# faverogian/diffusion-classifier

Measured on AMD Instinct MI355X. Metric: images classified/sec (node), CIFAR-10 10-class x 50-step ELBO scoring, higher is better.
Workload: dtype bf16; 1 GPU; cifar10-unet-10x50; classes=10, trials=50, forwards_per_image=500, input=uniform [-1,1], parallelism=single

## Files before the change

diffusion-classifier_amd/csrc/conv3_halo.hip:

```cpp
#include <stdlib.h>
#include "common.h"
#ifdef DC_STAMPS
static __device__ unsigned long long* g_stamps;
extern "C" void dc_debug_set_stamps(unsigned long long* p) { (void)hipMemcpyToSymbol(HIP_SYMBOL(g_stamps), &p, sizeof(p)); }
#define DC_STAMP(k) do { if (threadIdx.x == 0 && g_stamps) g_stamps[blockIdx.x * 8 + (k)] = __builtin_amdgcn_s_memtime(); } while (0)
static __device__ int g_halo_abl;
extern "C" void dc_debug_set_halo_abl(int v) { (void)hipMemcpyToSymbol(HIP_SYMBOL(g_halo_abl), &v, sizeof(v)); }
#define DC_HALO_ABL() __builtin_amdgcn_readfirstlane(g_halo_abl)
#else
#define DC_STAMP(k) do {} while (0)
#define DC_HALO_ABL() 0
#endif
#include "igemm_epilogue.h"
#include "epi_pn.h"

static __device__ unsigned g_pn_timeouts;
static __device__ chunk16 g_zero_page[16];
#include "conv3_halo_plan.h"
DC_CLOCK_DECL(conv3_halo)

template <typename T, int NW, int NTAP = 9, int MODE = 0, bool STG = false, bool PN = false, typename... TL>
__global__ __launch_bounds__(NW * 64, 2) void conv3_halo_kernel(const IgemmArgs a, const HaloGeom g, const TL... tl) {
  constexpr bool TAIL = sizeof...(TL) == 1;
  static_assert(sizeof...(TL) <= 1 && (!TAIL || (PN && NW == 4 && NTAP == 9 && MODE == 1 && sizeof(T) == 2)), "tail fold: the 16-bit 4-wave exchange form");
  static_assert(!PN || (MODE == 1 && NW == 4 && !STG) || ((MODE == 0 || MODE == 2) && NW == 8 && STG && NTAP == 9), "producer-side GroupNorm: one-image-per-patch forms, or 8x8 / 4x4 images");
  constexpr bool PNX = PN && NW == 4, PNL = PN && NW == 8;
  static_assert(!STG || NW == 8, "staggered loop: the 8-wave kernel");
  constexpr bool XB = MODE == 1, MOS = MODE == 2;
  using Cfg = HaloCfg<NW>;
  constexpr int EPC = Elem<T>::EPC;
  constexpr int BKE = 4 * EPC;
  constexpr int TM = 8, TN = 4;
  constexpr int NT = Cfg::NT, WLD = Cfg::WLD, WR = Cfg::WR, PD = Cfg::WR - 1;
  extern __shared__ __attribute__((aligned(16))) char smem[];
  char* const Wring = smem + 2 * Cfg::XBUF;

  DC_STAMP(0);
  const int t = threadIdx.x;
  const int lane = t & 63;
  const int wave = __builtin_amdgcn_readfirstlane(t >> 6);
  const int wm = wave >> 1, wn = wave & 1;
  const int lr = lane & 15, lq = lane >> 4;
  int tile_m, tile_n;
  if constexpr (PNX) {
    constexpr int LPH = NTAP == 4 ? 2 : 0;
    const int tnr = a.tiles_n >> LPH;
    const int kq = blockIdx.x >> 3;
    const int grp = ((kq >> (g.lpt + LPH)) << 3) + (blockIdx.x & 7);
    if (grp >= g.n_img * tnr) return;
    const int smp = grp / tnr;
    const int within = kq & ((1 << (g.lpt + LPH)) - 1);
    tile_n = __builtin_amdgcn_readfirstlane((within >> g.lpt) * tnr + grp - smp * tnr);
    tile_m = __builtin_amdgcn_readfirstlane((smp << g.lpt) + (within & ((1 << g.lpt) - 1)));
    asm volatile("" : "+s"(tile_m), "+s"(tile_n));
  } else if constexpr (XB) tile_of_block_scalar(a, tile_m, tile_n);
  else tile_of_block(a, tile_m, tile_n);
  constexpr bool UP4 = NTAP == 4;
  int phase = 0;
  if (UP4) { const int tn = a.tiles_n >> 2; phase = tile_n / tn; tile_n -= phase * tn; }
  const int pa = phase >> 1, pb = phase & 1;
  int tx = tile_m % g.tiles_x;
  int ty = (tile_m / g.tiles_x) % g.tiles_y;
  int ng = tile_m / (g.tiles_x * g.tiles_y);
  const int tw = 1 << g.ltw, th = 1 << g.lth;
  const int HW = g.H * g.W;
  const int HWs = a.upsample ? (g.H >> 1) * (g.W >> 1) : HW;
  const int Ctot = a.C0 + a.C1;
  const int c0chunks = a.C0 / BKE, nchunks = Ctot / BKE;

  constexpr int NXL = Cfg::NXL;
  int pp[NXL];
  const int xlx = t & 3;
  int* const tbl = reinterpret_cast<int*>(smem + Cfg::TBLOFF);
  if (t < (1 << g.lni)) {
    const int n = (ng << g.lni) + t;
    const bool vn = n < g.n_img;
    tbl[4 * t] = vn ? (a.map0 ? a.map0[n] : n) * HWs : -1;
    tbl[4 * t + 1] = (vn && a.src1) ? (a.map1 ? a.map1[n] : n) * HWs : -1;
    tbl[4 * t + 2] = (vn && a.src2) ? (a.map2 ? a.map2[n] : n) * HWs : -1;
  }
  auto piece_code = [&](int i, int* col = nullptr) -> int {
    const int hr = (i * NT + t) >> 2;
    int code = -1;
    if (col) *col = 0;
    if (i < g.nxl && hr < g.HR) {
      if constexpr (MOS) {
        const int hy = (int)(((float)hr + 0.5f) * g.inv_hw), hx = hr - hy * g.hw;
        const int cy = (int)(((float)hy + 0.5f) * g.inv_ch), ry = hy - cy * (th + 1);
        const int cx = (int)(((float)hx + 0.5f) * g.inv_cw), rx = hx - cx * (tw + 1);
        if (col) *col = hx;
        if (ry > 0 && rx > 0) code = (((cy << g.lmc) + cx) << 20) | ((ry - 1) * g.W + rx - 1);
      } else {
        const int img = (int)(((float)hr + 0.5f) * g.inv_hp), r = hr - img * g.hp;
        const int hy = (int)(((float)r + 0.5f) * g.inv_hw), hx = r - hy * g.hw;
        const int iy = ty * th + hy - 1, ix = tx * tw + hx - 1;
        if (col) *col = hx;
        if ((unsigned)iy < (unsigned)g.H && (unsigned)ix < (unsigned)g.W)
          code = (img << 20) | (a.upsample ? (iy >> 1) * (g.W >> 1) + (ix >> 1) : iy * g.W + ix);
      }
    }
    return code;
  };
  constexpr bool SWP = !STG;
#pragma unroll
  for (int i = 0; i < NXL; ++i) {
    int col;
    pp[i] = piece_code(i, &col);
    if constexpr (SWP) { if (pp[i] >= 0) pp[i] |= ((col >> g.sws) & 1) << 30; }
  }
  auto sw_of = [&](int pk) -> int { if constexpr (SWP) return (pk >> 30) & 1; else return 0; };
  constexpr int PKMASK = SWP ? 0x3FFFFFFF : -1;
  float* const brv = reinterpret_cast<float*>(smem + Cfg::GNOFF);
  constexpr bool STAGE_BRV = XB;
  if (STAGE_BRV && t < 128) {
    const int c = tile_n * 128 + t;
    float v = 0.f;
    if (c < a.Cout) {
      if (a.bias) v = a.bias[c];
      if (a.rowvec) v += a.rowvec[(size_t)(a.rowvec_map ? a.rowvec_map[ng] : ng) * a.rowvec_ld + c];
    }
    brv[t] = v;
  }
  if constexpr (PNX) {
    if (t >= 128 && t < 256) {
      const int c = tile_n * 128 + t - 128;
      brv[t] = a.pn_gamma[c];
      brv[t + 128] = a.pn_beta[c];
    }
  }
  __syncthreads();
  const char* zero = reinterpret_cast<const char*>(g_zero_page);
  constexpr bool XROW = STG && !XB;
  auto retarget = [&](int which) {
#pragma unroll
    for (int i = 0; i < NXL; ++i) {
      const int code = piece_code(i);
      int row = -1;
      if (code >= 0) {
        const int b = tbl[4 * (code >> 20) + which];
        if (b >= 0) row = b + (code & 0xFFFFF);
      }
      pp[i] = row;
    }
  };
  if constexpr (XROW) retarget(0);

  const T* xb0 = nullptr; const T* xb1 = nullptr; const T* xb2 = nullptr;
  int wvoff = 0, ldb0 = 0, ldb1 = 0, ldb2 = 0;
  if (XB) {
    ldb0 = a.ld0 * (int)sizeof(T); ldb1 = a.ld1 * (int)sizeof(T); ldb2 = a.ld2 * (int)sizeof(T);
    asm volatile("" : "+s"(ldb0), "+s"(ldb1), "+s"(ldb2));
    const int n = ng;
    const int s0 = __builtin_amdgcn_readfirstlane(a.map0 ? a.map0[n] : n);
    xb0 = reinterpret_cast<const T*>(a.src0) + (size_t)s0 * HWs * a.ld0;
    if (a.src1) { const int s1 = __builtin_amdgcn_readfirstlane(a.map1 ? a.map1[n] : n); xb1 = reinterpret_cast<const T*>(a.src1) + (size_t)s1 * HWs * a.ld1; }
    if (a.src2) { const int s2 = __builtin_amdgcn_readfirstlane(a.map2 ? a.map2[n] : n); xb2 = reinterpret_cast<const T*>(a.src2) + (size_t)s2 * HWs * a.ld2; }
  }
  if (XB || STG) {
    const int wrow0 = t >> 2;
    wvoff = (epi_wrow(wrow0, false) * a.Ktot + ((t & 3) ^ swz64(wrow0)) * EPC) * (int)sizeof(T);
  }
  auto rsrc_of = [](const void* base) { return __builtin_amdgcn_make_buffer_rsrc(const_cast<void*>(base), 0, 0x7fffffff, 0x00020000); };

  auto issue_x = [&](int cc, int i0 = 0, int i1 = 64) {
    const int which = cc >= nchunks ? 2 : (cc >= c0chunks ? 1 : 0);
    if constexpr (XB) {
      int ldb = ldb0, cb = cc;
      const T* xb = xb0;
      if (cc >= nchunks) { ldb = ldb2; cb = cc - nchunks; xb = xb2; }
      else if (cc >= c0chunks) { ldb = ldb1; cb = cc - c0chunks; xb = xb1; }
      const int cofs = cb * 64 + xlx * 16;
      const __amdgpu_buffer_rsrc_t rs = rsrc_of(xb);
      char* xs = smem + (cc & 1) * Cfg::XBUF + wave * 1024;
#pragma unroll
      for (int i = 0; i < NXL; ++i) {
        if (i < i0 || i >= i1) continue;
        int pk = pp[i];
        asm volatile("" : "+v"(pk));
        const int voff = pk < 0 ? -1 : (pk & PKMASK) * ldb + (cofs ^ (sw_of(pk) << 5));
        __builtin_amdgcn_raw_ptr_buffer_load_lds(rs, (lptr_t)(xs + i * (NT * 16)), 16, voff, 0, 0, 0);
      }
      return;
    } else {
    const T* src = reinterpret_cast<const T*>(which == 2 ? a.src2 : (which == 1 ? a.src1 : a.src0));
    const int ld = which == 2 ? a.ld2 : (which == 1 ? a.ld1 : a.ld0);
    const int coff = (which == 2 ? cc - nchunks : (which == 1 ? cc - c0chunks : cc)) * BKE + xlx * EPC;
    char* xs = smem + (cc & 1) * Cfg::XBUF + wave * 1024;
#pragma unroll
    for (int i = 0; i < NXL; ++i) {
      if (i < i0 || i >= i1) continue;
      int pk = pp[i];
      asm volatile("" : "+v"(pk));
      int rowi;
      if constexpr (XROW) rowi = pk;
      else {
        const int base = pk < 0 ? -1 : tbl[4 * ((pk & PKMASK) >> 20) + which];
        rowi = base < 0 ? -1 : base + (pk & 0xFFFFF);
      }
      const size_t e = (size_t)(rowi < 0 ? 0 : rowi) * ld + (coff ^ (sw_of(pk) << 1) * EPC);
      const char* gp = rowi < 0 ? zero : reinterpret_cast<const char*>(src + e);
      __builtin_amdgcn_global_load_lds((gptr_t)gp, (lptr_t)(xs + i * (NT * 16)), 16, 0, 0);
    }
    }
  };
  const int wtile0 = ((UP4 ? phase * (a.tiles_n >> 2) : 0) + tile_n) * 128 * a.Ktot;
  auto issue_w = [&](int cc, int tap, int slot) {
    if constexpr (XB || STG) {
      const int so = (wtile0 + tap * Ctot + cc * BKE) * (int)sizeof(T);
      const __amdgpu_buffer_rsrc_t wrs = rsrc_of(a.W);
#pragma unroll
      for (int i = 0; i < WLD; ++i)
        __builtin_amdgcn_raw_ptr_buffer_load_lds(wrs, (lptr_t)(Wring + slot * HALO_WST + i * (NT * 16) + wave * 1024), 16, wvoff,
                                                 __builtin_amdgcn_readfirstlane(so + i * 64 * a.Ktot * (int)sizeof(T)), 0, 0);
    } else {
      const T* wb = reinterpret_cast<const T*>(a.W) + (size_t)wtile0 + (size_t)tap * Ctot + (size_t)cc * BKE;
      int tt = t;
      asm volatile("" : "+v"(tt));
#pragma unroll
      for (int i = 0; i < WLD; ++i) {
        const int row = (i * NT + tt) >> 2;
        const int wro = epi_wrow(row, false) * a.Ktot + ((tt & 3) ^ swz64(row)) * EPC;
        __builtin_amdgcn_global_load_lds((gptr_t) reinterpret_cast<const char*>(wb + wro),
                                         (lptr_t)(Wring + slot * HALO_WST + i * (NT * 16) + wave * 1024), 16, 0, 0);
      }
    }
  };

  auto issue_w2 = [&](int e, int slot) {
    int tt = t;
    asm volatile("" : "+v"(tt));
#pragma unroll
    for (int i = 0; i < WLD; ++i) {
      const int row = (i * NT + tt) >> 2;
      const T* wp = reinterpret_cast<const T*>(a.W2) + (size_t)(tile_n * 128 + epi_wrow(row, false)) * a.C2 + ((tt & 3) ^ swz64(row)) * EPC + e * BKE;
      __builtin_amdgcn_global_load_lds((gptr_t) reinterpret_cast<const char*>(wp),
                                       (lptr_t)(Wring + slot * HALO_WST + i * (NT * 16) + wave * 1024), 16, 0, 0);
    }
  };
  const int nx = a.src2 ? a.C2 / BKE : 0;

  constexpr int NV = 3;
  int xlv[NV];
  {
    const int xx = lr & ((tw < 16 ? tw : 16) - 1);
    const int rowpart = ((lr >> g.ltw) * g.hw + (lr & (tw - 1))) * 64;
#pragma unroll
    for (int k = 0; k < NV; ++k) xlv[k] = rowpart + ((lq ^ (SWP ? (((xx + k + (UP4 ? pb : 0)) >> g.sws) & 1) << 1 : 0)) << 4);
  }
  int joff[TM];
#pragma unroll
  for (int j = 0; j < TM; ++j) {
    const int p = wm * 128 + j * 16;
    const int img = p >> (g.ltw + g.lth), py = (p >> g.ltw) & (th - 1), px = p & (tw - 1);
    const int o = MOS ? ((img >> g.lmc) * (th + 1) + py) * g.hw + (img & ((1 << g.lmc) - 1)) * (tw + 1) + px : img * g.hp + py * g.hw + px;
    joff[j] = __builtin_amdgcn_readfirstlane(o * 64);
  }
  const int woff0 = lds64_off(wn * 64 + lr, lq);

  f32x4 acc[TN][TM];
#pragma unroll
  for (int i = 0; i < TN; ++i)
#pragma unroll
    for (int j = 0; j < TM; ++j) acc[i][j] = f32x4{0.f, 0.f, 0.f, 0.f};

  constexpr int XD = HALO_XDEPTH;
  static_assert(XD >= 2 && XD <= TM, "pixel-fragment ring: 2 ... TM quads");
  const uint32_t lds0 = lds_addr_of(smem);
  const uint32_t waddr = lds_addr_of(Wring) + (uint32_t)woff0;
  auto mma_tap = [&](uint32_t wso, uint32_t xbo, int tapoff, auto kxc) {
    constexpr int kx = decltype(kxc)::value;
    chunk16 wf[TN], xq[XD];
    const uint32_t xu = lds0 + xbo + (uint32_t)tapoff;
    auto xread = [&](int j) { return ds_read16_async(xu + (uint32_t)joff[j] + (uint32_t)xlv[MOS ? ((kx + j) & 1) : kx]); };
    __builtin_amdgcn_sched_barrier(0);
    const uint32_t wa = waddr + wso;
    wf[0] = ds_read16_async_off<0>(wa);
    wf[1] = ds_read16_async_off<1024>(wa);
    wf[2] = ds_read16_async_off<2048>(wa);
    wf[3] = ds_read16_async_off<3072>(wa);
#pragma unroll
    for (int j = 0; j < XD; ++j) xq[j] = xread(j);
    auto group = [&](auto jc) {
      constexpr int j = decltype(jc)::value, q = j % XD;
      constexpr int fly = (TM - 1 - j) < (XD - 1) ? (TM - 1 - j) : (XD - 1);
      if constexpr (j == 0) lgkm_wait<fly>(wf[0], wf[1], wf[2], wf[3], xq[0]);
      else lgkm_wait<fly>(xq[q]);
      __builtin_amdgcn_sched_barrier(0);
#pragma unroll
      for (int i = 0; i < TN; ++i) acc[i][j] = Mma<T>::run(wf[i], xq[q], acc[i][j]);
      __builtin_amdgcn_sched_barrier(0);
      if constexpr (j + XD < TM) xq[q] = xread(j + XD);
    };
    group(IC<0>{}); group(IC<1>{}); group(IC<2>{}); group(IC<3>{}); group(IC<4>{}); group(IC<5>{}); group(IC<6>{}); group(IC<7>{});
    __builtin_amdgcn_sched_barrier(0);
  };

  DC_STAMP(1);
  if constexpr (STG) {
    const bool grpB = wave >= 4;
    const int abl = DC_HALO_ABL();
    int cur_which = 0;
    issue_x(0);
#pragma unroll
    for (int i = 0; i < PD; ++i) issue_w(0, i, i);
    hwait_vmcnt<0>();
    __builtin_amdgcn_s_barrier();
    if (grpB) __builtin_amdgcn_s_barrier();
    DC_CLOCK(0);
    chunk16 wf[TN], xf[TM / 2];
    uint32_t xaddr[TM];
#pragma unroll
    for (int j = 0; j < TM; ++j) xaddr[j] = lds0 + (uint32_t)(joff[j] + xlv[0]);
    for (int cc = 0; cc < nchunks; ++cc) {
      const bool side_next = cc + 1 == nchunks && nx > 0;
      const bool has_next = cc + 1 < nchunks || side_next;
      const int s0 = cc * NTAP;
      const uint32_t xbo = (uint32_t)(cc & 1) * Cfg::XBUF;
      if constexpr (XROW) {
        const int wnext = cc + 1 >= nchunks ? 2 : (cc + 1 >= c0chunks ? 1 : 0);
        if (has_next && wnext != cur_which) { retarget(wnext); cur_which = wnext; }
      }
      auto step = [&](auto tapc) {
        constexpr int tap = decltype(tapc)::value;
        constexpr int ky = UP4 ? (tap >> 1) : tap / 3, kx = UP4 ? (tap & 1) : tap - ky * 3;
        const uint32_t rowo = xbo + (uint32_t)(((ky + pa) * g.hw + pb) * 64);
        const uint32_t wso = (uint32_t)((s0 + tap) % WR) * HALO_WST;
        __builtin_amdgcn_s_barrier();
        __builtin_amdgcn_sched_barrier(0);
        if (!(abl & 2)) {
        wf[0] = ds_read16_async_off<0>(waddr + wso);
        wf[1] = ds_read16_async_off<1024>(waddr + wso);
        wf[2] = ds_read16_async_off<2048>(waddr + wso);
        wf[3] = ds_read16_async_off<3072>(waddr + wso);
#pragma unroll
        for (int j = 0; j < TM / 2; ++j) xf[j] = ds_read16_async_off<kx * 64>(xaddr[j] + rowo);
        }
        constexpr int t2 = tap + PD;
        if (!(abl & 4)) {
        if (t2 < NTAP) issue_w(cc, t2, (s0 + t2) % WR);
        else if (side_next) { if (t2 - NTAP < nx) issue_w2(t2 - NTAP, (s0 + t2) % WR); }
        else if (has_next) issue_w(cc + 1, t2 - NTAP, (s0 + t2) % WR);
        }
        __builtin_amdgcn_s_barrier();
        asm volatile("s_waitcnt lgkmcnt(0)" : "+v"(wf[0]), "+v"(wf[1]), "+v"(wf[2]), "+v"(wf[3]), "+v"(xf[0]), "+v"(xf[1]), "+v"(xf[2]), "+v"(xf[3]));
        __builtin_amdgcn_sched_barrier(0);
        if (!(abl & 1)) {
#pragma unroll
        for (int i = 0; i < TN; ++i) acc[i][0] = Mma<T>::run(wf[i], xf[0], acc[i][0]);
        }
        __builtin_amdgcn_sched_barrier(0);
        __builtin_amdgcn_sched_barrier(0);
        if (!(abl & 1)) {
#pragma unroll
        for (int j = 1; j < TM / 2; ++j)
#pragma unroll
          for (int i = 0; i < TN; ++i) acc[i][j] = Mma<T>::run(wf[i], xf[j], acc[i][j]);
        }
        __builtin_amdgcn_sched_barrier(0);
        __builtin_amdgcn_s_barrier();
        __builtin_amdgcn_sched_barrier(0);
        if (!(abl & 2)) {
#pragma unroll
        for (int j = 0; j < TM / 2; ++j) xf[j] = ds_read16_async_off<kx * 64>(xaddr[TM / 2 + j] + rowo);
        }
        constexpr int XP_A = UP4 ? (tap == 1 ? NXL : 0) : (tap == 1 ? 2 : (tap >= 2 && tap <= 6 ? 1 : 0));
        constexpr int XP_C = UP4 ? (tap == 0 ? NXL : 0) : (tap == 0 ? 2 : (tap <= 5 ? 1 : 0));
        if (has_next && !(abl & 12)) {
          if constexpr (UP4) { if (tap == 0) issue_x(cc + 1); }
          else if constexpr (tap == 0) issue_x(cc + 1, 0, 2);
          else if constexpr (tap <= 5) issue_x(cc + 1, tap + 1, tap + 2);
        }
        constexpr int XP_B = XP_C + (UP4 ? (tap == 2 ? NXL : 0) : (tap == 2 ? 2 : (tap >= 3 && tap <= 7 ? 1 : 0)));
        if (has_next) {
          if (tap == NTAP - 1 && side_next && nx < PD) hwait_vmcnt<0>();
          else hwait_vmcnt<(PD - 1) * WLD + XP_A + XP_B>();
        } else {
          constexpr int left = NTAP - 1 - tap;
          if constexpr (left > 0) hwait_vmcnt<((left - 1) < (PD - 1) ? (left - 1) : (PD - 1)) * WLD>();
        }
        __builtin_amdgcn_s_barrier();
        asm volatile("s_waitcnt lgkmcnt(0)" : "+v"(xf[0]), "+v"(xf[1]), "+v"(xf[2]), "+v"(xf[3]));
        __builtin_amdgcn_sched_barrier(0);
        if (!(abl & 1)) {
#pragma unroll
        for (int i = 0; i < TN; ++i) acc[i][TM / 2] = Mma<T>::run(wf[i], xf[0], acc[i][TM / 2]);
        }
        __builtin_amdgcn_sched_barrier(0);
        __builtin_amdgcn_sched_barrier(0);
        if (!(abl & 1)) {
#pragma unroll
        for (int j = 1; j < TM / 2; ++j)
#pragma unroll
          for (int i = 0; i < TN; ++i) acc[i][TM / 2 + j] = Mma<T>::run(wf[i], xf[j], acc[i][TM / 2 + j]);
        }
        __builtin_amdgcn_sched_barrier(0);
      };
      step(IC<0>{}); step(IC<1>{}); step(IC<2>{}); step(IC<3>{});
      if constexpr (NTAP == 9) { step(IC<4>{}); step(IC<5>{}); step(IC<6>{}); step(IC<7>{}); step(IC<8>{}); }
    }
    if (!grpB) __builtin_amdgcn_s_barrier();
    DC_CLOCK(1);
  } else {
  issue_x(0);
#pragma unroll
  for (int i = 0; i < PD; ++i) issue_w(0, i, i);
  constexpr int FLYL = (PD - 1) * WLD;
  DC_CLOCK(0);
  for (int cc = 0; cc < nchunks; ++cc) {
    const bool side_next = cc + 1 == nchunks && nx > 0;
    const bool has_next = cc + 1 < nchunks || side_next;
    const int s0 = cc * NTAP;
    const uint32_t xbo = (uint32_t)(cc & 1) * Cfg::XBUF;
    auto step = [&](auto tapc) {
      constexpr int tap = decltype(tapc)::value;
      if (has_next) {
        if (tap >= 1 && tap <= PD) hwait_vmcnt<FLYL + NXL>();
        else hwait_vmcnt<FLYL>();
      } else {
        constexpr int left = NTAP - 1 - tap;
        hwait_vmcnt<(left < PD - 1 ? left : PD - 1) * WLD>();
      }
      __builtin_amdgcn_s_barrier();
      constexpr int t2 = tap + PD;
      if (t2 < NTAP) issue_w(cc, t2, (s0 + t2) % WR);
      else if (side_next) { if (t2 - NTAP < nx) issue_w2(t2 - NTAP, (s0 + t2) % WR); }
      else if (has_next) issue_w(cc + 1, t2 - NTAP, (s0 + t2) % WR);
      if (tap == 0 && has_next) issue_x(cc + 1);

      const uint32_t wso = (uint32_t)((s0 + tap) % WR) * HALO_WST;
      constexpr int ky = UP4 ? (tap >> 1) : tap / 3, kx = UP4 ? (tap & 1) : tap - ky * 3;
      const int tapoff = ((ky + pa) * g.hw + kx + pb) * 64;
      mma_tap(wso, xbo, tapoff, IC<kx>{});
    };
    step(IC<0>{}); step(IC<1>{}); step(IC<2>{}); step(IC<3>{});
    if constexpr (NTAP == 9) { step(IC<4>{}); step(IC<5>{}); step(IC<6>{}); step(IC<7>{}); step(IC<8>{}); }
  }

  DC_CLOCK(1);
  }
  constexpr int FLY = (PD - 1) * WLD;
  {
    const int NSm = nchunks * NTAP;
    for (int e = 0; e < nx; ++e) {
      if (e == 0 && nx >= PD) hwait_vmcnt<FLY>();
      else hwait_vmcnt<0>();
      __builtin_amdgcn_s_barrier();
      if (e + PD < nx) issue_w2(e + PD, (NSm + e + PD) % WR);
      if (e + 1 < nx) issue_x(nchunks + e + 1);
      const uint32_t xbo = (uint32_t)((nchunks + e) & 1) * Cfg::XBUF;
      const uint32_t wso = (uint32_t)((NSm + e) % WR) * HALO_WST;
      const int tapoff = (g.hw + 1) * 64;
      mma_tap(wso, xbo, tapoff, IC<1>{});
    }
  }

  DC_STAMP(2);
  if constexpr (!XB) asm volatile("" : "+v"(tx), "+v"(ty), "+v"(ng), "+v"(tile_n));
  const int nw0 = min((ng << g.lni) + ((wm * 128) >> (g.ltw + g.lth)), g.n_img - 1);
  const int nw1 = min((ng << g.lni) + ((wm * 128 + 127) >> (g.ltw + g.lth)), g.n_img - 1);
  HaloQs qsfn;
  qsfn.nbase = ng << g.lni; qsfn.ltp = g.ltw + g.lth; qsfn.n_img = g.n_img; qsfn.tile_in_img = ty * g.tiles_x + tx; qsfn.wm = wm;
  qsfn.np = HW >= 128 ? HW >> 7 : 1;
  qsfn.padd = 0;
  if (UP4) { qsfn.padd = phase * qsfn.np; qsfn.np *= 4; }
  auto rowfn = [&](int j, EpiRow& r) {
    const int p = wm * 128 + j * 16 + lr;
    int n = (ng << g.lni) + (p >> (g.ltw + g.lth));
    r.ok = n < g.n_img;
    n = r.ok ? n : g.n_img - 1;
    const int py = (p >> g.ltw) & (th - 1), px = p & (tw - 1);
    const int rem = (ty * th + py) * g.W + tx * tw + px;
    r.samp = n;
    r.o = UP4 ? n * (4 * HW) + (2 * (ty * th + py) + pa) * (2 * g.W) + 2 * (tx * tw + px) + pb : n * HW + rem;
    r.r = (a.residual && a.res_map ? a.res_map[n] : n) * HW + rem;
  };
  if constexpr (PNL && MOS) {
    epi_direct_act<T, TM, DC_ACT_NONE, false, false>(a, acc, tile_n, wn, lq, nw0, nw1, rowfn, EpiNoPre(), qsfn, EpiNoBias(), EpiPnLocal4x4());
  } else if constexpr (PNL) {
    epi_direct_act<T, TM, DC_ACT_NONE, false, true>(a, acc, tile_n, wn, lq, nw0, nw1, rowfn, EpiNoPre(), qsfn, EpiNoBias(), EpiPnLocal8x8());
  } else if constexpr (PNX) {
    PnCtx pc;
    pc.sample = ng; pc.part = (UP4 ? phase * (HW >> 7) : 0) + ((ty * g.tiles_x + tx) << 1) + wm;
    pc.parts = (HW >> 7) << (UP4 ? 2 : 0); pc.tiles = 1 << (g.lpt + (UP4 ? 2 : 0));
    pc.qpg = (a.Cout / a.pn_groups) >> 2;
    pc.cnt = a.pn_cnt + (size_t)ng * (UP4 ? a.tiles_n >> 2 : a.tiles_n) + tile_n; pc.timeouts = &g_pn_timeouts;
    pc.gam = brv + 128 + wn * 64 + lq * 8; pc.bet = brv + 256 + wn * 64 + lq * 8;
    pc.scr = reinterpret_cast<float2*>(pc.tiles > 1 ? smem + wave * 4096 : smem + wn * 256);
    pc.flag = reinterpret_cast<int*>(brv + 384);
    pc.eps = a.pn_eps; pc.silu = a.pn_silu;
    if constexpr (TAIL) {
      PnTailCtx tc;
      tc.p = [](const PnTail& p, auto...) { return p; }(tl...);
      tc.zs = reinterpret_cast<float*>(smem);
      tc.wm = wm; tc.ltw = g.ltw; tc.lth = g.lth; tc.tx = tx; tc.ty = ty; tc.tiles_x = g.tiles_x; tc.lpt = g.lpt; tc.H = g.H; tc.W = g.W;
      epi_halo_pn<T>(a, acc, tile_n, wn, lq, rowfn, brv + wn * 64 + lq * 8, pc, tc);
    } else
    epi_halo_pn<T>(a, acc, tile_n, wn, lq, rowfn, brv + wn * 64 + lq * 8, pc);
  } else if constexpr (STAGE_BRV) {
    epi_direct_act<T, TM, DC_ACT_NONE, false, true>(a, acc, tile_n, wn, lq, nw0, nw1, rowfn, EpiNoPre(), qsfn, HaloLdsBias{brv + wn * 64 + lq * 8});
  } else {
    epi_direct_act<T, TM, DC_ACT_NONE, false, !MOS>(a, acc, tile_n, wn, lq, nw0, nw1, rowfn, EpiNoPre(), qsfn);
  }
  DC_STAMP(7);
}

struct ThinCfg {
  static constexpr int NT = 256, NXL = 6;
  static constexpr int XBUF = NXL * NT * 16;
  static constexpr int WBUF = 3 * NT * 16;
  static constexpr int TBLOFF = 2 * XBUF + 2 * WBUF;
  static constexpr int LDS = TBLOFF + 128;
  static constexpr int GNOFF = LDS, GNMAXC = 512;
  static constexpr int LDS_GN = GNOFF + 2 * GNMAXC * 4;
};

template <typename T, bool GN>
__global__ __launch_bounds__(256, 2) void conv3_thin_kernel(const IgemmArgs a, const HaloGeom g) {
  using Cfg = ThinCfg;
  constexpr int EPC = Elem<T>::EPC;
  constexpr int BKE = 4 * EPC;
  constexpr int TM = 4, NT = Cfg::NT, NXL = Cfg::NXL;
  extern __shared__ __attribute__((aligned(16))) char smem[];
  char* const Wl = smem + 2 * Cfg::XBUF;
  const int t = threadIdx.x;
  const int lane = t & 63;
  const int wave = __builtin_amdgcn_readfirstlane(t >> 6);
  const int lr = lane & 15, lq = lane >> 4;
  const int tile_m = blockIdx.x;
  const int tx = tile_m % g.tiles_x;
  const int ty = (tile_m / g.tiles_x) % g.tiles_y;
  const int ng = tile_m / (g.tiles_x * g.tiles_y);
  const int tw = 1 << g.ltw, th = 1 << g.lth;
  const int HW = g.H * g.W;
  const int Ctot = a.C0 + a.C1;
  const int c0chunks = a.C0 / BKE, nchunks = Ctot / BKE;

  int pp[NXL];
  const int xlx = t & 3;
  int* const tbl = reinterpret_cast<int*>(smem + Cfg::TBLOFF);
  if (t < (1 << g.lni)) {
    const int n = (ng << g.lni) + t;
    const bool vn = n < g.n_img;
    tbl[4 * t] = vn ? (a.map0 ? a.map0[n] : n) * HW : -1;
    tbl[4 * t + 1] = (vn && a.src1) ? (a.map1 ? a.map1[n] : n) * HW : -1;
  }
#pragma unroll
  for (int i = 0; i < NXL; ++i) {
    const int hr = (i * NT + t) >> 2;
    pp[i] = -1;
    if (i < g.nxl && hr < g.HR) {
      const int img = (int)(((float)hr + 0.5f) * g.inv_hp), r = hr - img * g.hp;
      const int hy = (int)(((float)r + 0.5f) * g.inv_hw), hx = r - hy * g.hw;
      const int iy = ty * th + hy - 1, ix = tx * tw + hx - 1;
      if ((unsigned)iy < (unsigned)g.H && (unsigned)ix < (unsigned)g.W) pp[i] = (img << 20) | (iy * g.W + ix);
    }
  }
  __syncthreads();
  const char* zero = reinterpret_cast<const char*>(g_zero_page);
  auto issue = [&](int cc) {
    const int which = cc >= c0chunks ? 1 : 0;
    const T* src = reinterpret_cast<const T*>(which ? a.src1 : a.src0);
    const int ld = which ? a.ld1 : a.ld0;
    const int coff = (which ? cc - c0chunks : cc) * BKE + xlx * EPC;
    char* xs = smem + (cc & 1) * Cfg::XBUF + wave * 1024;
#pragma unroll
    for (int i = 0; i < NXL; ++i) {
      int pk = pp[i];
      asm volatile("" : "+v"(pk));
      const int base = pk < 0 ? -1 : tbl[4 * (pk >> 20) + which];
      const size_t e = (size_t)(base < 0 ? 0 : base + (pk & 0xFFFFF)) * ld + coff;
      const char* gp = base < 0 ? zero : reinterpret_cast<const char*>(src + e);
      __builtin_amdgcn_global_load_lds((gptr_t)gp, (lptr_t)(xs + i * (NT * 16)), 16, 0, 0);
    }
    char* ws = Wl + (cc & 1) * Cfg::WBUF + wave * 1024;
#pragma unroll
    for (int i = 0; i < 3; ++i) {
      const int p = i * NT + t;
      const int tap = p >> 6, row = (p >> 2) & 15;
      const bool ok = tap < 9;
      const T* wp = reinterpret_cast<const T*>(a.W) + (size_t)row * a.Ktot + (size_t)(ok ? tap : 0) * Ctot + cc * BKE + ((p & 3) ^ swz64(row)) * EPC;
      __builtin_amdgcn_global_load_lds((gptr_t)(ok ? reinterpret_cast<const char*>(wp) : zero), (lptr_t)(ws + i * (NT * 16)), 16, 0, 0);
    }
  };
  const int xl = ((lr >> g.ltw) * g.hw + (lr & (tw - 1))) * 64 + lq * 16;
  int joff[TM];
#pragma unroll
  for (int j = 0; j < TM; ++j) {
    const int p = wave * 64 + j * 16;
    const int img = p >> (g.ltw + g.lth), py = (p >> g.ltw) & (th - 1), px = p & (tw - 1);
    joff[j] = __builtin_amdgcn_readfirstlane((img * g.hp + py * g.hw + px) * 64);
  }
  const int woff0 = lds64_off(lr, lq);
  f32x4 acc[TM];
#pragma unroll
  for (int j = 0; j < TM; ++j) acc[j] = f32x4{0.f, 0.f, 0.f, 0.f};

  float* const gnp = reinterpret_cast<float*>(smem + Cfg::GNOFF);
  if constexpr (GN) {
    if (ng < g.n_img)
      for (int c = t; c < Ctot; c += NT) {
        gnp[c] = a.gn_scale[(size_t)ng * Ctot + c];
        gnp[Ctot + c] = a.gn_shift[(size_t)ng * Ctot + c];
      }
    __builtin_amdgcn_s_waitcnt(0xC07F);
  }
  issue(0);
  for (int cc = 0; cc < nchunks; ++cc) {
    hwait_vmcnt<0>();
    __builtin_amdgcn_s_barrier();
    if (cc + 1 < nchunks) issue(cc + 1);
    if constexpr (GN) {
      const float* sc = gnp + cc * BKE + xlx * EPC;
      const float* sh = sc + Ctot;
      float scr[EPC], shr[EPC];
#pragma unroll
      for (int e = 0; e < EPC; ++e) { scr[e] = sc[e]; shr[e] = sh[e]; }
#pragma unroll
      for (int i = 0; i < NXL; ++i) {
        if (pp[i] >= 0) {
          chunk16* q = reinterpret_cast<chunk16*>(smem + (cc & 1) * Cfg::XBUF + (i * NT + t) * 16);
          float f[EPC];
          chunk_to_f<T>(*q, f);
#pragma unroll
          for (int e = 0; e < EPC; ++e) {
            float v = f[e] * scr[e] + shr[e];
            if (a.gn_silu) v = silu_t<T>(v);
            f[e] = v;
          }
          *q = f_to_chunk<T>(f);
        }
      }
      __builtin_amdgcn_s_waitcnt(0xC07F);
      __builtin_amdgcn_s_barrier();
    }
    const char* Xb = smem + (cc & 1) * Cfg::XBUF;
    const char* Wb = Wl + (cc & 1) * Cfg::WBUF;
#pragma unroll
    for (int tap = 0; tap < 9; ++tap) {
      const int ky = tap / 3, kx = tap - ky * 3;
      const int tapoff = (ky * g.hw + kx) * 64;
      const chunk16 wf = *reinterpret_cast<const chunk16*>(Wb + tap * 1024 + woff0);
#pragma unroll
      for (int j = 0; j < TM; ++j) {
        const chunk16 xf = *reinterpret_cast<const chunk16*>(Xb + (tapoff + joff[j]) + xl);
        acc[j] = Mma<T>::run(wf, xf, acc[j]);
      }
    }
  }
#pragma unroll
  for (int j = 0; j < TM; ++j) {
    const int p = wave * 64 + j * 16 + lr;
    const int n = (ng << g.lni) + (p >> (g.ltw + g.lth));
    if (n >= g.n_img) continue;
    const int py = (p >> g.ltw) & (th - 1), px = p & (tw - 1);
    const size_t o = ((size_t)n * HW + (ty * th + py) * g.W + tx * tw + px) * a.out_ld;
#pragma unroll
    for (int r = 0; r < 4; ++r) {
      const int c = lq * 4 + r;
      if (c < a.Cout) store_as(a.out, o + c, a.out_dtype, acc[j][r] + (a.bias ? a.bias[c] : 0.f));
    }
  }
}

bool dc_conv3_thin_applicable(const IgemmArgs& a, int dtype) {
  static const bool off = getenv("DCAMD_NO_THIN") != nullptr;
  if (off || a.taps != 9 || a.stride != 1 || a.upsample || a.act != DC_ACT_NONE || a.gate || a.rowvec || a.residual || a.src2) return false;
  if (a.gn_scale && a.C0 + a.C1 > ThinCfg::GNMAXC) return false;
  if (a.Cout > 16) return false;
  const int H = a.Hin, W = a.Win;
  if (H < 16 || W < 16 || (H & (H - 1)) || (W & (W - 1))) return false;
  if ((long long)a.M >= (1LL << 31)) return false;
  const int bke = 64 / dc_dtype_size(dtype);
  return a.C0 % bke == 0 && a.C1 % bke == 0;
}

bool dc_conv3_halo_applicable(const IgemmArgs& a, int dtype) {
  if (a.taps != 9 || a.stride != 1 || a.act != DC_ACT_NONE || a.gate) return false;
  const int H = a.Hin, W = a.Win;
  static const bool no_mosaic = getenv("DCAMD_NO_MOSAIC") != nullptr;
  const bool mosaic = !no_mosaic && H == 4 && W == 4 && !a.upsample;
  if (!mosaic && (H < 8 || W < 8 || (H & (H - 1)) || (W & (W - 1)))) return false;
  if ((long long)a.M >= (1LL << 31)) return false;
  const int bke = 64 / dc_dtype_size(dtype);
  if (a.C0 % bke || a.C1 % bke) return false;
  return true;
}

bool dc_conv3_up4_applicable(const IgemmArgs& a, int dtype) {
  if (a.taps != 9 || a.stride != 1 || !a.upsample || a.act != DC_ACT_NONE || a.gate || a.gn_scale || a.src2 || a.residual) return false;
  IgemmArgs lo = a;
  lo.upsample = 0; lo.Hin = a.Hin >> 1; lo.Win = a.Win >> 1;
  return dc_conv3_halo_applicable(lo, dtype);
}

IgemmArgs dc_conv3_up4_walked(const IgemmArgs& a0) {
  IgemmArgs a = a0;
  a.upsample = 0; a.Hin = a0.Hin >> 1; a.Win = a0.Win >> 1;
  a.Ktot = 4 * (a.C0 + a.C1);
  a.tiles_n = 4 * a0.tiles_n;
  a.n_fast = 0;
  return a;
}

HaloPlan dc_conv3_halo_plan(const IgemmArgs& a, int dtype, int n_img, bool up4) {
  HaloPlan pl;
  HaloGeom& g = pl.g;
  const int NW = dc_conv3_halo_waves(a.Hin, a.Win);
  HaloKey& k = pl.key;
  k = HaloKey{NW, up4 ? 4 : 9, 0, false, false};
  const bool fits = halo_geom(g, a.Hin, a.Win, n_img, NW * 64, NW * 64, NW == 4 ? HaloCfg<4>::NXL : HaloCfg<8>::NXL, NW == 8);
  const int ni = 1 << g.lni;
  if ((g.H < 8 || g.W < 8) && !g.mos) return halo_plan_fail(pl, "conv3_halo: %dx%d images need the 8-wave patch", g.H, g.W);
  g.sws = (g.ltw < 4 ? g.ltw : 4) - 2;
  const long long es = dc_dtype_size(dtype);
  g.xbuf = (ni == 1 && !g.mos && halo_xbuf_reach(a, dtype)) ? 1 : 0;
  k.MODE = g.mos ? 2 : (g.xbuf ? 1 : 0);
  if ((long long)a.tiles_n * 128 * a.Ktot >= (1LL << 31)) return halo_plan_fail(pl, "conv3_halo: weight matrix of %d x %d too large", a.tiles_n * 128, a.Ktot);
  if (!fits || g.nxl < 3) return halo_plan_fail(pl, "conv3_halo: halo of %d rows does not fit", g.HR);
  pl.tiles_m = ((n_img + ni - 1) / ni) * g.tiles_x * g.tiles_y;
  long long grid = (long long)pl.tiles_m * a.tiles_n;
  if (grid <= 0 || grid > 0x7fffffffLL) return halo_plan_fail(pl, "conv3_halo: bad grid %lld", grid);
  k.STG = NW == 8 && !up4 && !getenv("DCAMD_HALO_NO_STAG") && (long long)a.tiles_n * 128 * a.Ktot * es < (1LL << 31);
  if (a.pn_out) {
    if (NW == 4) {
      if (!g.xbuf || ni != 1) return halo_plan_fail(pl, "conv3_halo: producer-side GroupNorm needs the one-image-per-patch form");
      const long long groups = (long long)n_img * (up4 ? a.tiles_n >> 2 : a.tiles_n);
      grid = ((groups + 7) / 8 * 8) << (g.lpt + (up4 ? 2 : 0));
      if (grid > 0x7fffffffLL) return halo_plan_fail(pl, "conv3_halo: bad grid %lld", grid);
    } else {
      const bool i8 = !g.mos && !g.xbuf && g.H == 8 && g.W == 8 && ni == 8, i4 = g.mos && g.H == 4 && g.W == 4 && ni == 32;
      if (up4 || !(i8 || i4)) return halo_plan_fail(pl, "conv3_halo: producer-side GroupNorm on the 8-wave patch needs 8x8 or 4x4 images");
      if (!k.STG) return halo_plan_fail(pl, "conv3_halo: producer-side GroupNorm on 8x8 images needs the staggered loop");
    }
    k.PN = true;
  }
  pl.grid = (unsigned)grid;
  return pl;
}

using HaloKern = void (*)(const IgemmArgs, const HaloGeom);

template <typename T, int NW, int NTAP, int MODE, bool STG = false, bool PN = false>
static HaloKern halo_instance() {
  static bool attr_done = false;
  const HaloKern kern = conv3_halo_kernel<T, NW, NTAP, MODE, STG, PN>;
  if (!attr_done) {
    (void)hipFuncSetAttribute(reinterpret_cast<const void*>(kern), hipFuncAttributeMaxDynamicSharedMemorySize, HaloCfg<NW>::LDS);
    attr_done = true;
  }
  return kern;
}

template <typename T>
static HaloKern halo_kernel(const HaloKey& k) {
  auto is = [&](int nw, int ntap, int mode, bool stg = false, bool pn = false) {
    return k.NW == nw && k.NTAP == ntap && k.MODE == mode && k.STG == stg && k.PN == pn;
  };
  if (is(8, 4, 0)) return halo_instance<T, 8, 4, 0>();
  if (is(8, 9, 0)) return halo_instance<T, 8, 9, 0>();
  if (is(8, 9, 1)) return halo_instance<T, 8, 9, 1>();
  if (is(8, 4, 1)) return halo_instance<T, 8, 4, 1>();
  if (is(8, 9, 2)) return halo_instance<T, 8, 9, 2>();
  if (is(8, 4, 2)) return halo_instance<T, 8, 4, 2>();
  if (is(8, 9, 2, true, true)) return halo_instance<T, 8, 9, 2, true, true>();
  if (is(8, 9, 0, true, true)) return halo_instance<T, 8, 9, 0, true, true>();
  if (is(8, 9, 0, true)) return halo_instance<T, 8, 9, 0, true>();
  if (is(8, 9, 1, true)) return halo_instance<T, 8, 9, 1, true>();
  if (is(8, 9, 2, true)) return halo_instance<T, 8, 9, 2, true>();
  if (is(4, 4, 0)) return halo_instance<T, 4, 4, 0>();
  if (is(4, 9, 0)) return halo_instance<T, 4, 9, 0>();
  if (is(4, 9, 1)) return halo_instance<T, 4, 9, 1>();
  if (is(4, 4, 1)) return halo_instance<T, 4, 4, 1>();
  if (is(4, 4, 1, false, true)) return halo_instance<T, 4, 4, 1, false, true>();
  if (is(4, 9, 1, false, true)) return halo_instance<T, 4, 9, 1, false, true>();
  return nullptr;
}

int dc_conv3_halo_launch(const HaloPlan& pl, const IgemmArgs& a0, int dtype, bool up4, hipStream_t s) {
  if (pl.status != DC_OK) { dc_set_error("%s", pl.message); return pl.status; }
  IgemmArgs a = up4 ? dc_conv3_up4_walked(a0) : a0;
  a.tiles_m = pl.tiles_m;
  const HaloKey& k = pl.key;
  HaloKern kern = nullptr;
  const int rc = dc_by_dtype(dtype, "dc_igemm: dtype", [&](auto t) { kern = halo_kernel<decltype(t)>(k); return (int)DC_OK; });
  if (rc != DC_OK) return rc;
  if (!kern) { dc_set_error("conv3_halo: no instance <%d,%d,%d,%d,%d>", k.NW, k.NTAP, k.MODE, (int)k.STG, (int)k.PN); return DC_ERR_UNSUPPORTED; }
  hipLaunchKernelGGL(kern, dim3(pl.grid), dim3(k.NW * 64), k.NW == 4 ? HaloCfg<4>::LDS : HaloCfg<8>::LDS, s, a, pl.g);
  return dc_check_launch("dc_igemm(conv3_halo)");
}

template <typename T>
static int launch_tail(const HaloPlan& pl, const IgemmArgs& a, const PnTail& tl, hipStream_t s) {
  static bool attr_done = false;
  void (*kern)(const IgemmArgs, const HaloGeom, const PnTail) = conv3_halo_kernel<T, 4, 9, 1, false, true, PnTail>;
  if (!attr_done) {
    (void)hipFuncSetAttribute(reinterpret_cast<const void*>(kern), hipFuncAttributeMaxDynamicSharedMemorySize, HaloCfg<4>::LDS);
    attr_done = true;
  }
  hipLaunchKernelGGL(kern, dim3(pl.grid), dim3(256), HaloCfg<4>::LDS, s, a, pl.g, tl);
  return dc_check_launch("dc_conv3_pn_tail(conv3_halo)");
}

static_assert(2 * 256 * PN_TAIL_ZLD * 4 <= 2 * HaloCfg<4>::XBUF + HaloCfg<4>::WR * HALO_WST, "tail fold: the z image must fit the halo buffers and the W ring");

bool dc_conv3_halo_tail_ok(const IgemmArgs& a, const HaloPlan& pl, int dtype, int Co) {
  const HaloKey& k = pl.key;
  return pl.status == DC_OK && k.NW == 4 && k.NTAP == 9 && k.MODE == 1 && !k.STG && k.PN && (dtype == DC_BF16 || dtype == DC_F16) &&
         a.Cout == 128 && a.tiles_n == 1 && Co >= 1 && 9 * Co <= 32 && Co <= 3 && !a.out;
}

int dc_conv3_halo_tail_launch(const HaloPlan& pl, const IgemmArgs& a0, int dtype, const PnTail& tl, hipStream_t s) {
  if (pl.status != DC_OK) { dc_set_error("%s", pl.message); return pl.status; }
  if (!dc_conv3_halo_tail_ok(a0, pl, dtype, tl.Co)) { dc_set_error("dc_conv3_pn_tail: no tail instance for this problem"); return DC_ERR_UNSUPPORTED; }
  IgemmArgs a = a0;
  a.tiles_m = pl.tiles_m;
  return dtype == DC_BF16 ? launch_tail<__bf16>(pl, a, tl, s) : launch_tail<_Float16>(pl, a, tl, s);
}

constexpr int PN_MAX_TILES = 16;
bool dc_conv3_halo_pn_ok(const IgemmArgs& a, const HaloPlan& pl, bool up4) {
  static const bool off = getenv("DCAMD_NO_PN") != nullptr;
  if (off || a.src1 || (!up4 && a.upsample)) return false;
  if (pl.status != DC_OK || !pl.key.PN) return false;
  if (((1 << pl.g.lpt) << (up4 ? 2 : 0)) > PN_MAX_TILES) return false;
  if (a.Cout % 128 || a.pn_groups <= 0 || a.Cout % a.pn_groups) return false;
  const int cpg = a.Cout / a.pn_groups;
  return cpg == 4 || cpg == 8 || cpg == 16 || cpg == 32;
}

unsigned dc_conv3_halo_pn_timeouts() {
  unsigned v = 0, z = 0;
  if (hipMemcpyFromSymbol(&v, HIP_SYMBOL(g_pn_timeouts), sizeof(v)) != hipSuccess) return ~0u;
  if (v) (void)hipMemcpyToSymbol(HIP_SYMBOL(g_pn_timeouts), &z, sizeof(z));
  return v;
}

HaloPlan dc_conv3_thin_plan(const IgemmArgs& a, int n_img) {
  HaloPlan pl;
  pl.key = HaloKey{4, 9, 0, false, false};
  HaloGeom& g = pl.g;
  if (!halo_geom(g, a.Hin, a.Win, n_img, 256, ThinCfg::NT, ThinCfg::NXL, false)) return halo_plan_fail(pl, "conv3_thin: halo of %d rows does not fit", g.HR);
  const int ni = 1 << g.lni;
  const long long nblk = (long long)((n_img + ni - 1) / ni) * g.tiles_x * g.tiles_y;
  if (nblk <= 0 || nblk > 0x7fffffffLL) return halo_plan_fail(pl, "conv3_thin: bad grid %lld", nblk);
  if (a.gn_scale && ni != 1) return halo_plan_fail(pl, "conv3_thin: the fused GroupNorm needs one sample per patch");
  pl.tiles_m = (int)nblk; pl.grid = (unsigned)nblk;
  return pl;
}

template <typename T>
static int launch_thin(const HaloPlan& pl, const IgemmArgs& a, hipStream_t s) {
  static bool attr_done = false;
  const bool gn = a.gn_scale != nullptr;
  void (*kern)(const IgemmArgs, const HaloGeom) = gn ? conv3_thin_kernel<T, true> : conv3_thin_kernel<T, false>;
  const int lds = gn ? ThinCfg::LDS_GN : ThinCfg::LDS;
  if (!attr_done) {
    (void)hipFuncSetAttribute(reinterpret_cast<const void*>(conv3_thin_kernel<T, false>), hipFuncAttributeMaxDynamicSharedMemorySize, ThinCfg::LDS);
    (void)hipFuncSetAttribute(reinterpret_cast<const void*>(conv3_thin_kernel<T, true>), hipFuncAttributeMaxDynamicSharedMemorySize, ThinCfg::LDS_GN);
    attr_done = true;
  }
  hipLaunchKernelGGL(kern, dim3(pl.grid), dim3(ThinCfg::NT), lds, s, a, pl.g);
  return dc_check_launch("dc_igemm(conv3_thin)");
}

int dc_conv3_thin_launch(const IgemmArgs& a, int dtype, int n_img, hipStream_t s) {
  const HaloPlan pl = dc_conv3_thin_plan(a, n_img);
  if (pl.status != DC_OK) { dc_set_error("%s", pl.message); return pl.status; }
  return dc_by_dtype(dtype, "dc_igemm: dtype", [&](auto t) { return launch_thin<decltype(t)>(pl, a, s); });
}
```

diffusion-classifier_amd/csrc/conv3_halo_plan.h:

```cpp
#pragma once
#include <stdarg.h>
#include <stdio.h>
#include "conv3_halo.h"

static inline int ilog2(int v) { int l = 0; while ((1 << l) < v) ++l; return l; }

static inline bool halo_geom(HaloGeom& g, int H, int W, int n_img, int pix, int nt, int nxl_cap, bool mosaic_ok) {
  g.H = H; g.W = W; g.n_img = n_img;
  const int tw = W < 32 ? W : 32;
  int th = pix / tw; if (th > H) th = H;
  const int ni = pix / (tw * th);
  g.ltw = ilog2(tw); g.lth = ilog2(th); g.lni = ilog2(ni);
  g.tiles_x = W / tw; g.tiles_y = H / th;
  g.hw = tw + 2; g.hp = (th + 2) * g.hw; g.HR = ni * g.hp;
  g.mos = 0; g.lmc = 0; g.inv_ch = g.inv_cw = 0.f;
  if (mosaic_ok && (H < 8 || W < 8) && tw == W && th == H && ni >= 2) {
    g.mos = 1;
    g.lmc = (g.lni + 1) / 2;
    const int cols = 1 << g.lmc, rows = ni >> g.lmc;
    g.hw = cols * (tw + 1) + 1;
    g.hp = 0;
    g.HR = (rows * (th + 1) + 1) * g.hw;
    g.inv_ch = 1.0f / (float)(th + 1); g.inv_cw = 1.0f / (float)(tw + 1);
  }
  g.inv_hp = g.hp ? 1.0f / (float)g.hp : 0.f; g.inv_hw = 1.0f / (float)g.hw;
  g.xbuf = 0; g.sws = 0;
  g.lpt = ilog2(g.tiles_x * g.tiles_y);
  g.nxl = (g.HR * 4 + nt - 1) / nt;
  return g.nxl <= nxl_cap;
}

static inline bool halo_xbuf_reach(const IgemmArgs& a, int dtype) {
  const long long es = dc_dtype_size(dtype);
  const long long hws = (long long)(a.upsample ? (a.Hin >> 1) * (a.Win >> 1) : a.Hin * a.Win);
  const long long ldmax = a.ld0 > a.ld1 ? (a.ld0 > a.ld2 ? a.ld0 : a.ld2) : (a.ld1 > a.ld2 ? a.ld1 : a.ld2);
  return hws * ldmax * es < (1LL << 31) && (long long)a.tiles_n * 128 * a.Ktot * es < (1LL << 31);
}

struct HaloKey { int NW, NTAP, MODE; bool STG, PN; };

struct HaloPlan {
  HaloGeom g;
  int tiles_m = 0;
  unsigned grid = 0;
  HaloKey key{};
  int status = DC_OK;
  char message[112] = "";
};

__attribute__((format(printf, 2, 3))) static inline HaloPlan& halo_plan_fail(HaloPlan& pl, const char* fmt, ...) {
  pl.status = DC_ERR_SHAPE;
  va_list ap;
  va_start(ap, fmt);
  vsnprintf(pl.message, sizeof(pl.message), fmt, ap);
  va_end(ap);
  return pl;
}

static inline void halo_plan_ints(const HaloPlan& pl, int32_t* out) {
  const HaloGeom& g = pl.g;
  const int32_t v[14] = {1 << g.ltw, 1 << g.lth, 1 << g.lni, g.tiles_x, g.tiles_y, g.hw, g.HR, g.nxl, g.mos, g.xbuf, g.sws, g.lpt, pl.tiles_m, (int32_t)pl.grid};
  for (int i = 0; i < 14; ++i) out[i] = v[i];
}

HaloPlan dc_conv3_halo_plan(const IgemmArgs& walked, int dtype, int n_img, bool up4);
int dc_conv3_halo_launch(const HaloPlan& pl, const IgemmArgs& a, int dtype, bool up4, hipStream_t s);
bool dc_conv3_halo_pn_ok(const IgemmArgs& a, const HaloPlan& pl, bool up4);
HaloPlan dc_conv3_thin_plan(const IgemmArgs& a, int n_img);
bool dc_conv3_halo_tail_ok(const IgemmArgs& a, const HaloPlan& pl, int dtype, int Co);
int dc_conv3_halo_tail_launch(const HaloPlan& pl, const IgemmArgs& a, int dtype, const PnTail& tl, hipStream_t s);
int dc_pn_tail_combine_launch(float* pred, const float* ring, int n_img, int ltw, int lth, int tiles_x, int tiles_y, int H, int W, int Co, int ld,
                              hipStream_t s);
HaloPlan dc_conv3_ws_plan(const IgemmArgs& a, int n_img);
```

Measured before the change: 238.5 images/s.

## Stream side-input 1x1 chunks through dense LDS tiles with pipelined loads in halo conv

The skip/side-input (src2, 1x1) K-chunks of the non-staggered halo conv kernel now get their activation tiles staged into the halo LDS buffers as dense tiles, via a new issue_x2 path. These loads are issued ahead in a three-deep ring overlapped with the weight ring, and the last 3x3 chunk prefetches the first side tile instead of another halo. The goal is to remove the previous side-input loop's reliance on the already-loaded halo centre tap, so the residual-projection GEMM gets its own pipelined operand stream. It adds LDS reuse constraints and vmcnt bookkeeping that must stay consistent, plus optional timing-stamp macros for debugging.

```diff
diff --git a/diffusion-classifier_amd/csrc/conv3_halo.hip b/diffusion-classifier_amd/csrc/conv3_halo.hip
--- a/diffusion-classifier_amd/csrc/conv3_halo.hip
+++ b/diffusion-classifier_amd/csrc/conv3_halo.hip
@@ -3,13 +3,28 @@
 #ifdef DC_STAMPS
 static __device__ unsigned long long* g_stamps;
 extern "C" void dc_debug_set_stamps(unsigned long long* p) { (void)hipMemcpyToSymbol(HIP_SYMBOL(g_stamps), &p, sizeof(p)); }
+#ifdef DC_SIDE_STAMPS
+#define DC_STAMP(k) do { if (((k) < 3 || (k) == 7) && threadIdx.x == 0 && g_stamps) g_stamps[blockIdx.x * 8 + (k)] = __builtin_amdgcn_s_memtime(); } while (0)
+#define DC_SIDE_PUT(k, v) do { if (threadIdx.x == 0 && g_stamps) g_stamps[blockIdx.x * 8 + (k)] = (v); } while (0)
+#define DC_SIDE_T0() unsigned long long side_w = 0, side_t = 0; DC_SIDE_PUT(3, __builtin_amdgcn_s_memtime())
+#define DC_SIDE_W0() side_t = __builtin_amdgcn_s_memtime()
+#define DC_SIDE_W1() side_w += __builtin_amdgcn_s_memtime() - side_t
+#define DC_SIDE_T1() do { DC_SIDE_PUT(4, __builtin_amdgcn_s_memtime()); DC_SIDE_PUT(5, side_w); } while (0)
+#else
 #define DC_STAMP(k) do { if (threadIdx.x == 0 && g_stamps) g_stamps[blockIdx.x * 8 + (k)] = __builtin_amdgcn_s_memtime(); } while (0)
+#endif
 static __device__ int g_halo_abl;
 extern "C" void dc_debug_set_halo_abl(int v) { (void)hipMemcpyToSymbol(HIP_SYMBOL(g_halo_abl), &v, sizeof(v)); }
 #define DC_HALO_ABL() __builtin_amdgcn_readfirstlane(g_halo_abl)
 #else
 #define DC_STAMP(k) do {} while (0)
 #define DC_HALO_ABL() 0
+#endif
+#ifndef DC_SIDE_T0
+#define DC_SIDE_T0() do {} while (0)
+#define DC_SIDE_W0() do {} while (0)
+#define DC_SIDE_W1() do {} while (0)
+#define DC_SIDE_T1() do {} while (0)
 #endif
 #include "igemm_epilogue.h"
 #include "epi_pn.h"
@@ -238,6 +253,40 @@
     }
   };
   const int nx = a.src2 ? a.C2 / BKE : 0;
+  constexpr int NXD = HALO_SIDE_NXD, NTL = halo_side_ntiles(NW);
+  static_assert(NXD * NT * 16 == (NW / 2) * HALO_SIDE_TILE, "a side chunk is NW / 2 dense tiles");
+  auto side_pix = [&](int i, int tt, int* img = nullptr) -> int {
+    const int p = (NW == 4 ? i >> 1 : i) * 128 + (NW == 4 ? (i & 1) * 64 : 0) + (tt >> 2);
+    if (img) *img = p >> (g.ltw + g.lth);
+    return (ty * th + ((p >> g.ltw) & (th - 1))) * g.W + tx * tw + (p & (tw - 1));
+  };
+  auto side_row = [&](int i, int tt) -> int {
+    int img;
+    const int pix = side_pix(i, tt, &img);
+    const int base = tbl[4 * img + 2];
+    return base < 0 ? -1 : base + pix;
+  };
+  auto issue_x2 = [&](int e, int i0 = 0, int i1 = NXD) {
+    int tt = t;
+    asm volatile("" : "+v"(tt));
+    const int tb = (nchunks & 1) * (NTL / 2) + e * (NW / 2);
+#pragma unroll
+    for (int i = 0; i < NXD; ++i) {
+      if (i < i0 || i >= i1) continue;
+      const int wmi = NW == 4 ? i >> 1 : i, sub = NW == 4 ? i & 1 : 0;
+      const int lc = (tt & 3) ^ swz64(sub * 64 + (tt >> 2));
+      char* const ls = smem + ((tb + wmi) % NTL) * HALO_SIDE_TILE + sub * (HALO_SIDE_TILE / 2) + wave * 1024;
+      if constexpr (XB) {
+        const __amdgpu_buffer_rsrc_t rs = rsrc_of(xb2);
+        const int voff = side_pix(i, tt) * ldb2 + e * 64 + lc * 16;
+        __builtin_amdgcn_raw_ptr_buffer_load_lds(rs, (lptr_t)ls, 16, voff, 0, 0, 0);
+      } else {
+        const int rowi = side_row(i, tt);
+        const char* gp = rowi < 0 ? zero : reinterpret_cast<const char*>(reinterpret_cast<const T*>(a.src2) + (size_t)rowi * a.ld2 + e * BKE + lc * EPC);
+        __builtin_amdgcn_global_load_lds((gptr_t)gp, (lptr_t)ls, 16, 0, 0);
+      }
+    }
+  };
 
   constexpr int NV = 3;
   int xlv[NV];
@@ -267,11 +316,8 @@
   static_assert(XD >= 2 && XD <= TM, "pixel-fragment ring: 2 ... TM quads");
   const uint32_t lds0 = lds_addr_of(smem);
   const uint32_t waddr = lds_addr_of(Wring) + (uint32_t)woff0;
-  auto mma_tap = [&](uint32_t wso, uint32_t xbo, int tapoff, auto kxc) {
-    constexpr int kx = decltype(kxc)::value;
+  auto mma_step = [&](uint32_t wso, auto xread) {
     chunk16 wf[TN], xq[XD];
-    const uint32_t xu = lds0 + xbo + (uint32_t)tapoff;
-    auto xread = [&](int j) { return ds_read16_async(xu + (uint32_t)joff[j] + (uint32_t)xlv[MOS ? ((kx + j) & 1) : kx]); };
     __builtin_amdgcn_sched_barrier(0);
     const uint32_t wa = waddr + wso;
     wf[0] = ds_read16_async_off<0>(wa);
@@ -293,6 +339,11 @@
     };
     group(IC<0>{}); group(IC<1>{}); group(IC<2>{}); group(IC<3>{}); group(IC<4>{}); group(IC<5>{}); group(IC<6>{}); group(IC<7>{});
     __builtin_amdgcn_sched_barrier(0);
+  };
+  auto mma_tap = [&](uint32_t wso, uint32_t xbo, int tapoff, auto kxc) {
+    constexpr int kx = decltype(kxc)::value;
+    const uint32_t xu = lds0 + xbo + (uint32_t)tapoff;
+    mma_step(wso, [&](int j) { return ds_read16_async(xu + (uint32_t)joff[j] + (uint32_t)xlv[MOS ? ((kx + j) & 1) : kx]); });
   };
 
   DC_STAMP(1);
@@ -414,7 +465,7 @@
     auto step = [&](auto tapc) {
       constexpr int tap = decltype(tapc)::value;
       if (has_next) {
-        if (tap >= 1 && tap <= PD) hwait_vmcnt<FLYL + NXL>();
+        if (tap >= 1 && tap <= PD) { if (NTAP == 9 && side_next) hwait_vmcnt<FLYL + NXD>(); else hwait_vmcnt<FLYL + NXL>(); }
         else hwait_vmcnt<FLYL>();
       } else {
         constexpr int left = NTAP - 1 - tap;
@@ -425,7 +476,7 @@
       if (t2 < NTAP) issue_w(cc, t2, (s0 + t2) % WR);
       else if (side_next) { if (t2 - NTAP < nx) issue_w2(t2 - NTAP, (s0 + t2) % WR); }
       else if (has_next) issue_w(cc + 1, t2 - NTAP, (s0 + t2) % WR);
-      if (tap == 0 && has_next) issue_x(cc + 1);
+      if (tap == 0 && has_next) { if (NTAP == 9 && side_next) issue_x2(0); else issue_x(cc + 1); }
 
       const uint32_t wso = (uint32_t)((s0 + tap) % WR) * HALO_WST;
       constexpr int ky = UP4 ? (tap >> 1) : tap / 3, kx = UP4 ? (tap & 1) : tap - ky * 3;
@@ -439,7 +490,7 @@
   DC_CLOCK(1);
   }
   constexpr int FLY = (PD - 1) * WLD;
-  {
+  if constexpr (STG) {
     const int NSm = nchunks * NTAP;
     for (int e = 0; e < nx; ++e) {
       if (e == 0 && nx >= PD) hwait_vmcnt<FLY>();
@@ -452,6 +503,34 @@
       const int tapoff = (g.hw + 1) * 64;
       mma_tap(wso, xbo, tapoff, IC<1>{});
     }
+  } else if (nx > 0) {
+    const int NSm = nchunks * NTAP;
+    uint32_t sl = waddr;
+    asm volatile("" : "+v"(sl));
+    sl += lds0 - lds_addr_of(Wring) - (uint32_t)(wn * 64 * 64);
+    const int tb = (nchunks & 1) * (NTL / 2) + wm;
+    DC_SIDE_T0();
+    for (int e = 0; e < nx; ++e) {
+      DC_SIDE_W0();
+      if (e == 0) { if (nx >= PD) hwait_vmcnt<FLY>(); else hwait_vmcnt<0>(); }
+      else if (e + PD - 1 < nx) hwait_vmcnt<WLD + NXD>();
+      else if (e + 1 < nx) hwait_vmcnt<NXD>();
+      else hwait_vmcnt<0>();
+      __builtin_amdgcn_s_barrier();
+      DC_SIDE_W1();
+      if (e == 0) {
+        issue_x2(1);
+        if (PD < nx) issue_w2(PD, (NSm + PD) % WR);
+        if (2 < nx) issue_x2(2);
+      } else {
+        if (e + PD < nx) issue_w2(e + PD, (NSm + e + PD) % WR);
+        if (e + 2 < nx) issue_x2(e + 2);
+      }
+      const uint32_t wso = (uint32_t)((NSm + e) % WR) * HALO_WST;
+      const uint32_t xs = sl + (uint32_t)((tb + e * (NW / 2)) % NTL) * HALO_SIDE_TILE;
+      mma_step(wso, [&](int j) { return ds_read16_async(xs + (uint32_t)(j * 16 * 64)); });
+    }
+    DC_SIDE_T1();
   }
 
   DC_STAMP(2);
diff --git a/diffusion-classifier_amd/csrc/conv3_halo_plan.h b/diffusion-classifier_amd/csrc/conv3_halo_plan.h
--- a/diffusion-classifier_amd/csrc/conv3_halo_plan.h
+++ b/diffusion-classifier_amd/csrc/conv3_halo_plan.h
@@ -37,6 +37,23 @@
   return hws * ldmax * es < (1LL << 31) && (long long)a.tiles_n * 128 * a.Ktot * es < (1LL << 31);
 }
 
+constexpr int HALO_SIDE_TILE = 8192;
+constexpr int HALO_SIDE_NXD = 4;
+__host__ __device__ constexpr int halo_side_ntiles(int nw) { return 2 * (nw == 4 ? HaloCfg<4>::XBUF : HaloCfg<8>::XBUF) / HALO_SIDE_TILE; }
+static_assert(2 * HaloCfg<4>::XBUF % HALO_SIDE_TILE == 0 && 2 * HaloCfg<8>::XBUF % HALO_SIDE_TILE == 0, "the halo buffers are whole dense tiles");
+static_assert(halo_side_ntiles(4) >= 3 * 2 && halo_side_ntiles(8) >= 3 * 4 && halo_side_ntiles(4) / 2 >= 2 && halo_side_ntiles(8) / 2 >= 4,
+              "three side chunks in flight, chunk 0 inside one halo buffer");
+__host__ __device__ inline int halo_side_tile(int nw, int nchunks, int e, int wm) {
+  const int T = halo_side_ntiles(nw);
+  return ((nchunks & 1) * (T / 2) + e * (nw / 2) + wm) % T;
+}
+__host__ __device__ inline int halo_side_issue_step(int e) { return e == 0 ? -1 : (e <= 2 ? 0 : e - 2); }
+__host__ __device__ inline int halo_side_fly(int nw, int e, int nx) {
+  const int WLD = nw == 4 ? HaloCfg<4>::WLD : HaloCfg<8>::WLD, PD = (nw == 4 ? HaloCfg<4>::WR : HaloCfg<8>::WR) - 1;
+  if (e == 0) return nx >= PD ? (PD - 1) * WLD : 0;
+  return (e + PD - 1 < nx ? WLD : 0) + (e + 1 < nx ? HALO_SIDE_NXD : 0);
+}
+
 struct HaloKey { int NW, NTAP, MODE; bool STG, PN; };
 
 struct HaloPlan {
```

Measured after the change: 238.6 images/s, median of 2. No clear change (+0.0%).
